# SleepingShell/verkle-kzg

Measured on AMD Instinct MI355X. Metric: width-256 commits/sec + 2^20-pt MSM ms at 1/2/4/8 GPU; achieved HBM GB/s, higher is better.
Workload: dtype u32; 1 GPU; single 2^20-point bls12_381 G1 Pippenger MSM (configs[1]); n_points=1048576, curve=bls12_381, parallelism=one GPU, exchange=none, window_bits=16, windows=7, radix=327680, radix_form=5 * 2^16, terms_per_point=2

## Files before the change

verkle-kzg_amd/csrc/ctx.hpp:

```cpp
#pragma once
#include <hip/hip_runtime.h>

#include <functional>
#include <map>
#include <memory>
#include <mutex>
#include <string>
#include <vector>

#include "../../include/vc_msm.h"

#define VK_CHECK_HIP(expr)                              \
    do {                                                \
        hipError_t e_ = (expr);                         \
        if (e_ != hipSuccess) {                         \
            vk::last_hip_error() = e_;                  \
            return e_ == hipErrorOutOfMemory ? VC_E_OOM : VC_E_HIP; \
        }                                               \
    } while (0)

#define VK_TRY(expr)            \
    do {                        \
        int s_ = (expr);        \
        if (s_ != VC_OK) return s_; \
// ... 94 lines not shown
    int win_ok = 0, win_c = 0, win_W = 0, win_ts = 0, win_m = 1;
    int win_limbs = 1;
    int win_pair = 0;
    DevBuf win;
    Table* lead = nullptr;
    int lead_k = 0, lead_c = 0;
    Table() = default;
    Table(const Table&) = delete;
    Table& operator=(const Table&) = delete;
    ~Table() { delete lead; }
};

enum WsSlot {
    WS_DIGITS = 0,
    WS_COUNTS,
    WS_OFFSETS,
    WS_CURSOR,
    WS_SORTED,
    WS_BUCKETS,
    WS_CARRY,
    WS_THROUGH,
    WS_OWNER,
    WS_OWNER_B,
    WS_SEG,
    WS_WIN,
    WS_SCAN_TMP,
    WS_SCALARS,
    WS_OUT,
    WS_MISC,
    WS_TREE,
    WS_TAIL,
    WS_PIECE,
    WS_SP_RP,
    WS_SP_COLS,
    WS_SP_SC,
    WS_SP_CNT,
    WS_SP_EOFF,
    WS_SP_OFF,
    WS_SP_ROWS,
    WS_SP_XY,
    WS_SP_INF,
    WS_SP_RC,
    WS_SP_CHUNKS,
    WS_CARRY2,
    WS_NXT,
    WS_NXT2,
    WS_CHAIN,
    WS_GLV_SC,
    WS_GLV_FLAG,
    WS_RAW_B,
    WS_SP_ITEMS,
    WS_NORM_CNT,
    WS_NORM_TOT,
    WS_COUNT_
};

struct Lane {
    hipStream_t st;
    DevBuf* ws;
    PinBuf* pin;
};

struct PendingTimer {
    hipEvent_t a, b;
    std::string name;
};

}

struct vc_ctx {
    int curve = 0;
    int device = 0;
    uint64_t uid = 0;
    hipStream_t stream = nullptr;
    hipStream_t own_stream = nullptr;
    hipStream_t side_stream = nullptr;
    std::recursive_mutex mu;
    std::vector<vk::Table*> tables;
    vk::DevBuf ws[vk::WS_COUNT_];
    vk::DevBuf ws2[vk::WS_COUNT_];
    vk::PinBuf pin[2];
    vk::PinBuf pin_io;
    vk::PinBuf pin_small;
    vk::PinBuf pin_norm;
    vk::PinBuf pin_y;
    vk::PinBuf pin_mp;
    vk::PinBuf pin_ipa;
    vk::PinBuf pin_verkle;
    vk::PinBuf pin_verkle2;
    vk::PinBuf pin_verkle_lv[2];
    vk::PinBuf pin_norm_vk;
    vk::PinBuf pin_sparse_ck;
    vk::PinBuf pin_sparse_ch;
    std::multimap<size_t, void*> pool_free;
    size_t pool_bytes = 0;
    bool timing = false;
    int opt_shared_windows = 1;
    size_t opt_msm_chunk = size_t(1) << 27;
    int opt_host_chunks = 2;
    uint32_t fb_lanes = 0;
    uint32_t small_epoch = 0;
    uint32_t tail_epoch = 0;
    uint32_t norm_vk_parity = 0;
    struct {
        int c, W, terms, m, shared;
    } plan = {0, 0, 0, 0, 0};
// ... 114 lines not shown
```

verkle-kzg_amd/csrc/msm.hip:

```cpp
#include <hip/hip_runtime.h>

#include <atomic>
#include <chrono>
#include <immintrin.h>
#include <cstdio>
#include <hipcub/hipcub.hpp>

#include <algorithm>
#include <type_traits>
#include <cstdlib>
#include <cstring>
#include <functional>
#include <mutex>
#include <set>
#include <utility>
#include <vector>

#include "ctx.hpp"
#include "host/pool.hpp"
#include "ec.hpp"
#include "msm_tail.hpp"
#include "ec29.hpp"

namespace vk {
// ... 200 lines not shown
        if (b0 + k < bins) {
            loff[b0 + k] = run;
            lcur[b0 + k] = run;
            run += counts[(size_t)(bin0 + b0 + k) * nblk + slot];
        }
    if (t == blockDim.x - 1) loff[bins] = part[t];
    __syncthreads();
    const uint32_t fmask = (1u << FB) - 1;
    const uint32_t lo = blockIdx.x * chunk, hi = min(lo + chunk, n);
    auto put = [&](uint32_t i, int w, int32_t d) {
        if (d != 0 && w >= wb) {
            const uint32_t b = (uint32_t)(d < 0 ? -d : d) - 1;
            const uint32_t p = atomicAdd(
                &lcur[(stride ? (uint32_t)w / wps : (uint32_t)(w - wb)) * NBC + (b >> FB) - bin0], 1u);
            stage[p] = sort_pack<uint32_t>(b & fmask, stride ? src.pt(i) + ((uint32_t)w % wps) * stride : i, d < 0, FB);
        }
    };
    if constexpr (std::is_same<Src, RadixDigits>::value) {
        constexpr int PRE = 4, WMAX = 8;
        if (we - src.w0 <= WMAX) {
            for (uint32_t i0 = lo + t; i0 < hi; i0 += PRE * blockDim.x) {
                int32_t dg[PRE][WMAX];
#pragma unroll
                for (int k = 0; k < PRE; k++) {
                    const uint32_t i = i0 + (uint32_t)k * blockDim.x;
#pragma unroll
                    for (int j = 0; j < WMAX; j++)
                        dg[k][j] = (i < hi && src.w0 + j < we) ? src.dig[(size_t)(src.w0 + j) * src.nv + i] : 0;
                }
#pragma unroll
                for (int k = 0; k < PRE; k++) {
                    const uint32_t i = i0 + (uint32_t)k * blockDim.x;
                    if (i >= hi) break;
#pragma unroll
                    for (int j = 0; j < WMAX; j++)
                        if (src.w0 + j < we) put(i, src.w0 + j, dg[k][j]);
                }
            }
        } else {
            for (uint32_t i = lo + t; i < hi; i += blockDim.x) src(i, c, we, [&](int w, int32_t d) { put(i, w, d); });
        }
    } else {
        for (uint32_t i = lo + t; i < hi; i += blockDim.x) src(i, c, we, [&](int w, int32_t d) { put(i, w, d); });
    }
    __syncthreads();
    const uint32_t grp = t >> 4, sub = t & 15, ngrp = blockDim.x >> 4;
    for (uint32_t g = grp; g < bins; g += ngrp) {
        const uint32_t l0 = loff[g], len = loff[g + 1] - l0;
        const uint32_t gb = base[(size_t)(bin0 + g) * nblk + slot];
        for (uint32_t j = sub; j < len; j += 16) tmp[gb + j] = stage[l0 + j];
    }
}

template <class T>
__global__ void __launch_bounds__(1024) k_sort_fine(const T* __restrict__ tmp, const uint32_t* __restrict__ base,
                                                   uint32_t nblk, uint32_t bins, uint32_t FB,
                                                   uint32_t* __restrict__ offsets, uint32_t* __restrict__ sorted,
                                                   uint32_t* __restrict__ zero_word, uint32_t cap, uint32_t regs_ok) {
    __shared__ uint32_t h[256], x[256];
    extern __shared__ uint32_t stage[];
    const uint32_t g = blockIdx.x, F = 1u << FB, t = threadIdx.x;
    const bool cnt_lane = t < 256;
    if (zero_word != nullptr && g == 0 && t == 0) *zero_word = 0;
    const uint32_t start = base[(size_t)g * nblk];
    const uint32_t end = base[(size_t)(g + 1) * nblk];
    if (cnt_lane) h[t] = 0;
    __syncthreads();
    constexpr uint32_t RMAX = 16;
    T er[RMAX];
    const bool regs = regs_ok != 0 && cap != 0 && end - start <= cap && end - start <= RMAX * blockDim.x;
    if (regs) {
#pragma unroll
        for (uint32_t k = 0; k < RMAX; k++) {
            const uint32_t p = start + t + k * blockDim.x;
            er[k] = p < end ? tmp[p] : T(0);
        }
#pragma unroll
        for (uint32_t k = 0; k < RMAX; k++)
            if (start + t + k * blockDim.x < end) atomicAdd(&h[sort_fine_of<T>(er[k], FB)], 1u);
    } else {
        constexpr uint32_t RH = 4;
        for (uint32_t p0 = start + t; p0 < end; p0 += RH * blockDim.x) {
            T e[RH];
#pragma unroll
            for (uint32_t k = 0; k < RH; k++) {
                const uint32_t p = p0 + k * blockDim.x;
                e[k] = p < end ? tmp[p] : T(0);
            }
#pragma unroll
            for (uint32_t k = 0; k < RH; k++)
                if (p0 + k * blockDim.x < end) atomicAdd(&h[sort_fine_of<T>(e[k], FB)], 1u);
        }
    }
    __syncthreads();
    const uint32_t v = cnt_lane ? h[t] : 0u;
    if (cnt_lane) x[t] = v;
    __syncthreads();
    for (uint32_t o = 1; o < 256; o <<= 1) {
        const uint32_t a = (cnt_lane && t >= o) ? x[t - o] : 0u;
        __syncthreads();
        if (cnt_lane) x[t] += a;
        __syncthreads();
    }
    const uint32_t excl = cnt_lane ? x[t] - v : 0u;
    if (t < F) offsets[(size_t)g * F + t] = start + excl;
    if (g == bins - 1 && t == 0) offsets[(size_t)bins * F] = end;
    __syncthreads();
    if (cnt_lane) h[t] = excl;
    __syncthreads();
    constexpr uint32_t RS = 4;
    if (regs) {
#pragma unroll
        for (uint32_t k = 0; k < RMAX; k++)
            if (start + t + k * blockDim.x < end) stage[atomicAdd(&h[sort_fine_of<T>(er[k], FB)], 1u)] = sort_entry_of<T>(er[k], FB);
        __syncthreads();
        for (uint32_t p = t; p < end - start; p += blockDim.x) sorted[start + p] = stage[p];
        return;
    }
    if (end - start <= cap) {
        for (uint32_t p0 = start + t; p0 < end; p0 += RS * blockDim.x) {
            T e[RS];
            uint32_t pos[RS];
#pragma unroll
            for (uint32_t k = 0; k < RS; k++) {
                const uint32_t p = p0 + k * blockDim.x;
                e[k] = p < end ? tmp[p] : T(0);
            }
#pragma unroll
            for (uint32_t k = 0; k < RS; k++)
                if (p0 + k * blockDim.x < end) pos[k] = atomicAdd(&h[sort_fine_of<T>(e[k], FB)], 1u);
#pragma unroll
            for (uint32_t k = 0; k < RS; k++)
                if (p0 + k * blockDim.x < end) stage[pos[k]] = sort_entry_of<T>(e[k], FB);
        }
        __syncthreads();
        for (uint32_t p = t; p < end - start; p += blockDim.x) sorted[start + p] = stage[p];
        return;
    }
    for (uint32_t p0 = start + t; p0 < end; p0 += RS * blockDim.x) {
        T e[RS];
        uint32_t pos[RS];
#pragma unroll
        for (uint32_t k = 0; k < RS; k++) {
            const uint32_t p = p0 + k * blockDim.x;
            e[k] = p < end ? tmp[p] : T(0);
        }
#pragma unroll
        for (uint32_t k = 0; k < RS; k++)
            if (p0 + k * blockDim.x < end) pos[k] = start + atomicAdd(&h[sort_fine_of<T>(e[k], FB)], 1u);
#pragma unroll
        for (uint32_t k = 0; k < RS; k++)
            if (p0 + k * blockDim.x < end) sorted[pos[k]] = sort_entry_of<T>(e[k], FB);
    }
}

template <class FC, class BT, class = void>
struct is_affn : std::false_type {};
template <class FC, class BT>
struct is_affn<FC, BT, std::void_t<typename FC::AffN>> : std::is_same<BT, typename FC::AffN> {};
template <class FC, class BT, class = void>
struct is_affp : std::false_type {};
template <class FC, class BT>
struct is_affp<FC, BT, std::void_t<typename FC::AffP>> : std::is_same<BT, typename FC::AffP> {};
template <class C, class BT>
struct is_fbe : std::is_same<BT, FbE<C>> {};

static uint32_t acc_merge() {
    static const uint32_t v = getenv("VKZG_ACC_MERGE") ? (uint32_t)atoi(getenv("VKZG_ACC_MERGE")) : 0u;
    return v;
}

template <class T>
__device__ __forceinline__ T shfl_down1(const T& v) {
    static_assert(sizeof(T) % 4 == 0, "");
    constexpr int NW = (int)(sizeof(T) / 4);
    uint32_t w[NW];
    __builtin_memcpy(w, &v, sizeof w);
#pragma unroll
    for (int k = 0; k < NW; k++) w[k] = (uint32_t)__shfl_down((int)w[k], 1);
    T r;
    __builtin_memcpy(&r, w, sizeof w);
    return r;
}

template <class C, class BT = typename C::Aff>
__global__ void __launch_bounds__(256) VK_ACC_OCC k_msm_accumulate(
    const BT* __restrict__ bases, const BT* __restrict__ phi, uint32_t nphi,
    const uint32_t* __restrict__ sorted, const uint32_t* __restrict__ offsets, uint32_t NBtot, uint32_t M,
    typename Fast29<C>::type::Acc* __restrict__ buckets, typename Fast29<C>::type::Acc* __restrict__ carry_in,
    uint8_t* __restrict__ through, typename Fast29<C>::type::Acc* __restrict__ owner_piece,
    uint32_t* __restrict__ owner_bucket, uint32_t* __restrict__ chain_max, uint32_t merge,
    unsigned long long* __restrict__ clk) {
    using FC = typename Fast29<C>::type;
    using Aff = BT;
    uint32_t t = blockIdx.x * blockDim.x + threadIdx.x;
    const uint32_t L = offsets[NBtot];
    uint32_t k = t * M;
    if (k >= L) return;
    const bool stamp = clk != nullptr && t == 0;
    if (stamp) {
        clk[0] = __builtin_amdgcn_s_memtime();
        clk[1] = __builtin_amdgcn_s_memrealtime();
    }
    uint32_t e = min(k + M, L);
    owner_bucket[t] = NONE;
    through[t] = 0;
    uint32_t lo = 0, hi = NBtot;
    while (hi - lo > 1) {
        uint32_t mid = (lo + hi) >> 1;
        if (offsets[mid] <= k) lo = mid;
        else hi = mid;
    }
    uint32_t b = lo;
    uint32_t bend = offsets[b + 1];
    bool left_open = offsets[b] < k;
    typename FC::Acc acc = FC::zero();
    auto base_of = [&](uint32_t j) -> const Aff* { return j < nphi ? bases + j : phi + (j - nphi); };
    constexpr bool SN = is_affn<FC, BT>::value;
    constexpr bool SP = is_affp<FC, BT>::value;
    constexpr bool FBE = is_fbe<C, BT>::value;
    using Pre = std::conditional_t<SN || SP || FBE, typename FC::Aff, Aff>;
    auto fetch = [&](uint32_t id) -> Pre {
        if constexpr (FBE) {
            return base_of(id & 0x7fffffffu)->u;
        } else if constexpr (SP) {
            const Aff* r = bases + 2 * (size_t)(id & 0x7fffffffu) + (id >> 31);
            typename FC::Aff a;
            a.x = r->x;
            a.y = r->y;
            return a;
        } else {
            const Aff* b = base_of(id & 0x7fffffffu);
            if constexpr (SN) {
                typename FC::Aff a;
                a.x = b->x;
                a.y = *reinterpret_cast<const decltype(a.y)*>(reinterpret_cast<const char*>(&b->y) +
                                                              ((id >> 31) ? sizeof(a.y) : 0u));
                return a;
            } else {
                return *b;
            }
        }
    };
    uint32_t idx = sorted[k];
    Pre P = fetch(idx);
    uint32_t my_through = 0, own_b = NONE;
    while (true) {
        uint32_t cur = idx;
        typename FC::Aff Q;
        if constexpr (SN || SP || FBE) Q = P;
        else Q = FC::load(&P);
        if (k + 1 < e) {
            idx = sorted[k + 1];
            P = fetch(idx);
        }
        acc = FC::madd(acc, Q, !SN && !SP && (cur >> 31) != 0);
        k++;
        if (k == bend || k == e) {
            bool right_open = (k == e) && (bend > e);
            if (!left_open && !right_open) {
                buckets[b] = acc;
            } else if (left_open) {
                carry_in[t] = acc;
                my_through = right_open ? 2 : 1;
                through[t] = (uint8_t)my_through;
                if (!right_open) {
                    const uint32_t L = t - offsets[b] / M;
                    if (L >= 2) atomicMax(chain_max, L);
                }
            } else {
                owner_piece[t] = acc;
                owner_bucket[t] = b;
                own_b = b;
            }
            if (k == e) break;
            left_open = false;
            acc = FC::zero();
            do {
                b++;
                bend = offsets[b + 1];
            } while (bend <= k);
        }
    }
    if (stamp) {
        clk[2] = __builtin_amdgcn_s_memtime();
        clk[3] = __builtin_amdgcn_s_memrealtime();
    }
#ifdef VKZG_ACC_MERGE_BUILD
    if (merge) {
        const typename FC::Acc mine = my_through == 1 ? carry_in[t] : FC::zero();
        const typename FC::Acc nxt = shfl_down1(mine);
        const uint32_t nth = (uint32_t)__shfl_down((int)my_through, 1);
        if (own_b != NONE && (threadIdx.x & 63u) != 63u && nth == 1) {
            buckets[own_b] = FC::add(acc, nxt);
            owner_bucket[t] = NONE;
        }
    }
#else
    (void)merge;
    (void)my_through;
    (void)own_b;
#endif
}

template <class C>
__global__ void __launch_bounds__(256) k_fast_store(const FAcc<C>* __restrict__ a, uint32_t n,
                                                   const uint32_t* __restrict__ offsets, typename C::Acc* __restrict__ o) {
    const uint32_t i = blockIdx.x * blockDim.x + threadIdx.x;
    if (i < n && offsets[i + 1] > offsets[i]) o[i] = Fast29<C>::type::store(a[i]);
}

template <class C>
__global__ void __launch_bounds__(256) k_to_fast(const typename C::Aff* __restrict__ in, size_t n,
                                                typename C::Aff* __restrict__ out) {
    const size_t i = (size_t)blockIdx.x * blockDim.x + threadIdx.x;
    if (i >= n) return;
    Fast29<C>::type::pack_aff(in[i], out + i);
}
template <class C>
__global__ void __launch_bounds__(256) k_to_limbs(const typename C::Aff* __restrict__ in, size_t n,
                                                 typename Fast29<C>::type::Aff* __restrict__ out) {
    using FC = typename Fast29<C>::type;
    const size_t i = (size_t)blockIdx.x * blockDim.x + threadIdx.x;
    if (i >= n) return;
    typename C::Aff packed;
    FC::pack_aff(in[i], &packed);
    out[i] = FC::load(&packed);
}

template <class C>
__global__ void __launch_bounds__(256) k_to_limbs_n(const typename C::Aff* __restrict__ in, size_t n,
                                                   typename Fast29<C>::type::AffN* __restrict__ out) {
    using FC = typename Fast29<C>::type;
    const size_t i = (size_t)blockIdx.x * blockDim.x + threadIdx.x;
// ... 399 lines not shown
    t->win_pair = (pair && !packed) ? 1 : 0;
    VK_TRY(t->win.ensure((size_t)W * 2 * n * (packed ? sizeof(Aff) : t->win_pair ? 2 * sizeof(FP) : sizeof(FA))));
    Table cur;
    DevBuf nxt, acc;
    VK_TRY(nxt.ensure(n * sizeof(Aff)));
    VK_TRY(acc.ensure(n * sizeof(Acc)));
    FA* win = t->win.as<FA>();
    const unsigned g = (unsigned)((n + 255) / 256);
    for (int w = 0; w < W; w++) {
        const Aff* src = t->bases.as<Aff>();
        if (w > 0) {
            VK_LAUNCH(ctx, "win_next", (k_win_next<C>), g, 256, 0, w == 1 ? t->bases.as<Aff>() : cur.bases.as<Aff>(),
                      t->inf.as<uint8_t>(), (uint32_t)n, w == W - 1 ? c - ts : c, mul, acc.as<Acc>());
            VK_TRY(table_from_acc(ctx, &cur, acc.p, n));
            src = cur.bases.as<Aff>();
        }
        VK_LAUNCH(ctx, "glv_phi", (k_glv_phi<C>), g, 256, 0, src, (uint32_t)n, bls_fq_mont(GLV_BETA), nxt.as<Aff>());
        if (packed) {
            Aff* wp = t->win.as<Aff>();
            VK_LAUNCH(ctx, "to_fast", (k_to_fast<C>), g, 256, 0, src, n, wp + (size_t)w * 2 * n);
            VK_LAUNCH(ctx, "to_fast", (k_to_fast<C>), g, 256, 0, nxt.as<Aff>(), n, wp + (size_t)w * 2 * n + n);
        } else if (t->win_pair) {
            FP* wp = t->win.as<FP>();
            VK_LAUNCH(ctx, "to_limbs", (k_to_limbs_p<C>), g, 256, 0, src, n, wp + 2 * ((size_t)w * 2 * n));
            VK_LAUNCH(ctx, "to_limbs", (k_to_limbs_p<C>), g, 256, 0, nxt.as<Aff>(), n, wp + 2 * ((size_t)w * 2 * n + n));
        } else {
            VK_LAUNCH(ctx, "to_limbs", (k_to_limbs_n<C>), g, 256, 0, src, n, win + (size_t)w * 2 * n);
            VK_LAUNCH(ctx, "to_limbs", (k_to_limbs_n<C>), g, 256, 0, nxt.as<Aff>(), n, win + (size_t)w * 2 * n + n);
        }
    }
    VK_CHECK_HIP(hipStreamSynchronize(ctx->stream));
    t->win_ok = 1;
    t->win_c = c;
    t->win_W = W;
    t->win_ts = ts;
    t->win_m = (int)mul;
    return VC_OK;
}

static int coarse_st_lds_attr(const void* fn, int device) {
    static std::mutex mu;
    static std::set<std::pair<const void*, int>> done;
    std::lock_guard<std::mutex> lk(mu);
    if (done.count({fn, device})) return VC_OK;
    VK_CHECK_HIP(hipFuncSetAttribute(fn, hipFuncAttributeMaxDynamicSharedMemorySize, 152 * 1024));
    done.insert({fn, device});
    return VC_OK;
}

template <class Src>
static int sort_entries(vc_ctx* ctx, Lane L, Src src, uint32_t nv, int c, int wb, int we, uint32_t FB,
                        uint32_t NBC, uint32_t nblk, uint32_t chunk, uint32_t stride, uint32_t wps, size_t ncnt,
                        uint32_t* counts, uint32_t* base, void* tmp, uint32_t* offsets, uint32_t* sorted,
                        uint32_t* zero_word, bool coarse_stage = false, bool counts_ready = false,
                        uint32_t sets_split = 1) {
    hipStream_t st = L.st;
    if (stride && wps == 0) return VC_E_INVALID;
    const uint32_t bins = (stride ? ((uint32_t)we + wps - 1) / wps : (uint32_t)(we - wb)) * NBC;
    const size_t lds = (size_t)bins * 4;
    if (lds > 64 * 1024) return VC_E_INVALID;
    if (ncnt != (size_t)bins * nblk + 1) return VC_E_INVALID;
    const uint64_t emax = stride ? (uint64_t)std::min<uint32_t>((uint32_t)we, wps) * stride : (uint64_t)nv;
    const bool narrow = emax <= (1ull << (31 - FB));
    const uint32_t sblk = chunk >= 4096 ? 1024 : 256;
    if (!counts_ready)
        VK_LAUNCH_ON(ctx, st, "msm_sort_hist", (k_sort_hist<Src>), nblk, sblk, lds, src, nv, c, wb, we, FB, NBC,
                     nblk, stride, wps, chunk, counts);
    size_t tmp_bytes = 0;
    VK_CHECK_HIP(hipcub::DeviceScan::ExclusiveSum(nullptr, tmp_bytes, counts, base, ncnt, st));
    VK_TRY(L.ws[WS_SCAN_TMP].ensure(tmp_bytes));
    {
        hipEvent_t ev = nullptr;
        if (ctx->timing) ctx->timer_begin("msm_scan", &ev, st);
        VK_CHECK_HIP(hipcub::DeviceScan::ExclusiveSum(L.ws[WS_SCAN_TMP].p, tmp_bytes, counts, base, ncnt, st));
        if (ctx->timing) ctx->timer_end("msm_scan", ev, st);
    }
    static const int fine_env = getenv("VKZG_SORT_FINE_BLOCK") ? atoi(getenv("VKZG_SORT_FINE_BLOCK")) : 0;
    const uint64_t total = (uint64_t)nv * (uint32_t)(we - wb);
    int fblk = fine_env == 256 || fine_env == 1024 ? fine_env : (total / bins >= (1u << 15) ? 1024 : 256);
    static const int stage_env = getenv("VKZG_SORT_STAGE") ? atoi(getenv("VKZG_SORT_STAGE")) : 1;
    static const uint32_t fine_regs = !(getenv("VKZG_SORT_FINE_REGS") && atoi(getenv("VKZG_SORT_FINE_REGS")) == 0);
    uint32_t cap = 0;
    if (stage_env && total / bins <= 12000) {
        cap = 16384;
        if (fine_env == 0) fblk = 1024;
    }
    const uint32_t nsplit = (stride && sets_split > 1 && wb == 0 && (uint32_t)we == sets_split * wps) ? sets_split : 1;
    const uint32_t bins_l = bins / nsplit;
    const uint32_t wl = (uint32_t)(we - wb) / nsplit;
    const size_t st_lds = ((size_t)2 * bins_l + 1 + (size_t)chunk * wl) * 4;
    const bool staged = coarse_stage && narrow && st_lds <= 152 * 1024;
    if (staged) {
        VK_TRY(coarse_st_lds_attr(reinterpret_cast<const void*>(&k_sort_coarse_st<Src>), ctx->device));
        for (uint32_t s = 0; s < nsplit; s++) {
            Src ss = src;
            const int wbs = nsplit > 1 ? (int)(s * wps) : wb, wes = nsplit > 1 ? (int)((s + 1) * wps) : we;
            if constexpr (std::is_same<Src, RadixDigits>::value) ss.w0 = wbs;
            VK_LAUNCH_ON(ctx, st, "msm_sort_coarse", k_sort_coarse_st<Src>, nblk, 1024, st_lds, ss, nv, c, wbs, wes, FB,
                         NBC, nblk, stride, wps, chunk, counts, base, static_cast<uint32_t*>(tmp), s * bins_l, bins_l);
        }
        VK_LAUNCH_ON(ctx, st, "msm_sort_fine", k_sort_fine<uint32_t>, bins, fblk, cap * 4,
                     static_cast<const uint32_t*>(tmp), base, nblk, bins, FB, offsets, sorted, zero_word, cap, fine_regs);
    } else if (narrow) {
        VK_LAUNCH_ON(ctx, st, "msm_sort_coarse", (k_sort_coarse<Src, uint32_t>), nblk, sblk, lds, src, nv, c, wb, we,
                     FB, NBC, nblk, stride, wps, chunk, base, static_cast<uint32_t*>(tmp));
        VK_LAUNCH_ON(ctx, st, "msm_sort_fine", k_sort_fine<uint32_t>, bins, fblk, cap * 4,
                     static_cast<const uint32_t*>(tmp), base, nblk, bins, FB, offsets, sorted, zero_word, cap, fine_regs);
    } else {
        VK_LAUNCH_ON(ctx, st, "msm_sort_coarse", (k_sort_coarse<Src, uint64_t>), nblk, sblk, lds, src, nv, c, wb, we,
                     FB, NBC, nblk, stride, wps, chunk, base, static_cast<uint64_t*>(tmp));
        VK_LAUNCH_ON(ctx, st, "msm_sort_fine", k_sort_fine<uint64_t>, bins, fblk, cap * 4,
                     static_cast<const uint64_t*>(tmp), base, nblk, bins, FB, offsets, sorted, zero_word, cap, fine_regs);
    }
    return VC_OK;
}

static bool win_pair_on() {
    static const int env = getenv("VKZG_WIN_PAIR") ? atoi(getenv("VKZG_WIN_PAIR")) : 1;
    return env != 0;
}

static int glv_window(size_t nv) {
    if (nv >= (1u << 19)) return 16;
    if (nv >= (1u << 15)) return 13;
    return 10;
}
static int glv_window_shared(size_t nv) {
    static const int env = getenv("VKZG_MSM_C") ? atoi(getenv("VKZG_MSM_C")) : 0;
    if (env >= 8 && env <= 20) return env;
    return glv_window(nv);
}
static int top_shortfall(int c, int total) {
    const int W = (total + c - 1) / c;
    return c - (total - c * (W - 1));
}
static int choose_window(size_t n, int total) {
    int c0 = 5;
    if (n >= (1u << 19)) c0 = 16;
    else if (n >= (1u << 17)) c0 = 15;
    else if (n >= (1u << 15)) c0 = 13;
    else if (n >= (1u << 12)) c0 = 11;
    else if (n >= (1u << 9)) c0 = 9;
    else if (n >= 64) c0 = 7;
    static const int env = getenv("VKZG_MSM_TOPFIT") ? atoi(getenv("VKZG_MSM_TOPFIT")) : 1;
    if (!env || top_shortfall(c0, total) <= 2) return c0;
    int best = c0;
    double best_cost = 0.0;
    for (int c = std::max(4, c0 - 5); c <= std::min(16, c0 + 2); c++) {
        if (top_shortfall(c, total) > 2) continue;
        const double W = (total + c - 1) / c;
        const double cost = W * (double)n + 2.0 * W * (double)(1u << (c - 1));
        if (best == c0 || cost < best_cost) best = c, best_cost = cost;
    }
    return best;
}

template <class C>
struct MsmSlice {
    using Acc = typename C::Acc;
    Lane L{};
    int c = 0, wb = 0, we = 0, W = 0;
    bool shared = false;
    int top_f = 0;
    uint32_t m = 1;
    int sets = 1;
// ... 60 lines not shown
    const bool resid_sets = sl.shared || Wr <= 8;
    const uint32_t nU = (Lseg > 1 && resid_sets && (resid_env == 1 || (resid_env == 2 && sl.shared))) ? Lseg : 1;
    const uint32_t Tmax = (uint32_t)((maxL + M - 1) / M);
    hipStream_t st = L.st;

    const uint32_t lgNB = (uint32_t)c - 1;
    uint32_t FB = lgNB < 8 ? lgNB : 8;
    uint32_t chunk = SORT_CHUNK;
    if (sl.m > 1) {
        FB = lgNB < 7 ? lgNB : 7;
        chunk = 8192;
    }
    static const int chunk_env = getenv("VKZG_SORT_CHUNK") ? atoi(getenv("VKZG_SORT_CHUNK")) : 0;
    static const int fb_env = getenv("VKZG_SORT_FB") ? atoi(getenv("VKZG_SORT_FB")) : 0;
    static const int cstage_env = getenv("VKZG_SORT_CSTAGE") ? atoi(getenv("VKZG_SORT_CSTAGE")) : 1;
    bool cstage = false;
    if (sl.m > 1 && sl.shared && cstage_env) {
        const uint64_t bins_l = (uint64_t)(NB >> FB);
        const uint32_t Wl = (uint32_t)W / (uint32_t)Wr;
        const uint64_t room = (152u * 1024 / 4 > 2 * bins_l + 1) ? 152u * 1024 / 4 - 2 * bins_l - 1 : 0;
        uint32_t ch = 1u << 12;
        while (ch > 1024 && (uint64_t)ch * Wl > room) ch >>= 1;
        if ((uint64_t)ch * Wl <= room) {
            chunk = ch;
            cstage = true;
        }
    }
    if (sl.m == 1 && !sl.shared && cstage_env && FB > 1 && load / (NB >> FB) > 12000) FB--;
    if (chunk_env >= 256) chunk = (uint32_t)chunk_env;
    static const int bin_lg = getenv("VKZG_SORT_BIN_LG") ? atoi(getenv("VKZG_SORT_BIN_LG")) : 16;
    while (sl.shared && sl.m == 1 && FB > 1 && (load >> bin_lg) > (size_t)(NB >> FB)) FB--;
    while (sl.shared && sl.m == 1 && FB > 1 && (NB >> FB) < 256) FB--;
    if (fb_env >= 1 && fb_env <= (int)std::min<uint32_t>(lgNB, 8)) FB = (uint32_t)fb_env;
    const uint32_t NBC = NB >> FB;
    const uint32_t nblk = (uint32_t)((nv + chunk - 1) / chunk);
    if (sl.m == 1 && cstage_env) {
        const uint64_t per_blk = (uint64_t)chunk * (uint32_t)(sl.we - sl.wb), bins_all = (uint64_t)Wr * NBC;
        const uint64_t lds_b = (2 * bins_all + 1 + per_blk) * 4;
        cstage = per_blk >= 4096 && (per_blk >= 10 * bins_all || lds_b <= 64 * 1024);
    }
    const size_t ncnt = (size_t)Wr * NBC * nblk + 1;

    DevBuf* ws = L.ws;
    VK_TRY(ws[WS_DIGITS].ensure(maxL * 8));
    VK_TRY(ws[WS_COUNTS].ensure(ncnt * 4));
    VK_TRY(ws[WS_CURSOR].ensure(ncnt * 4));
    VK_TRY(ws[WS_OFFSETS].ensure((size_t)(NBtot + 1) * 4));
    VK_TRY(ws[WS_SORTED].ensure(maxL * 4));
    VK_TRY(ws[WS_BUCKETS].ensure((size_t)NBtot * sizeof(RAcc)));
    VK_TRY(ws[WS_CARRY].ensure((size_t)(Tmax + 8) * sizeof(RAcc)));
    VK_TRY(ws[WS_THROUGH].ensure((size_t)(Tmax + 8)));
    VK_TRY(ws[WS_OWNER].ensure((size_t)(Tmax + 8) * sizeof(RAcc)));
    VK_TRY(ws[WS_OWNER_B].ensure((size_t)(Tmax + 8) * 4));
    VK_TRY(ws[WS_SEG].ensure((size_t)S * Wr * sizeof(RAcc)));
    VK_TRY(ws[WS_TREE].ensure((size_t)S * Wr * sizeof(RAcc)));
    VK_TRY(ws[WS_WIN].ensure((size_t)Wr * msm_tail_plan(S, (uint32_t)Wr, J, nU, Fast29<C>::type::quad, Lseg == 1).slots *
                             sizeof(RAcc)));
    const size_t tail_bytes = ((size_t)Wr * (J + nU) * sizeof(Acc) + 15) & ~(size_t)15;
    VK_TRY(ws[WS_TAIL].ensure(tail_bytes + 16));

    sl.NB = NB;
    sl.NBtot = NBtot;
    sl.Tmax = Tmax;
    sl.M = M;
    sl.Lseg = Lseg;
    sl.S = S;
    sl.J = J;
    sl.nU = nU;
    sl.offsets = ws[WS_OFFSETS].as<uint32_t>();
    sl.tail_bytes = tail_bytes;
    sl.chain_max = sl.chain_dst ? sl.chain_dst : reinterpret_cast<uint32_t*>(ws[WS_TAIL].as<uint8_t>() + tail_bytes);
    sl.through = ws[WS_THROUGH].as<uint8_t>();
    sl.owner_b = ws[WS_OWNER_B].as<uint32_t>();
    sl.buckets = sl.bucket_dst ? sl.bucket_dst : ws[WS_BUCKETS].as<RAcc>();
    sl.carry = ws[WS_CARRY].as<RAcc>();
    sl.owner = ws[WS_OWNER].as<RAcc>();
    sl.seg = ws[WS_SEG].as<RAcc>();
    sl.rs = ws[WS_TREE].as<RAcc>();
    sl.bsum_part = ws[WS_WIN].as<RAcc>();
    sl.tail = ws[WS_TAIL].as<Acc>();

    bool counts_ready = false;
    static const bool timing = getenv("VKZG_HOST_TIMING") && atoi(getenv("VKZG_HOST_TIMING")) != 0;
    if (timing)
        sl.t_launch0 =
            std::chrono::duration<double, std::micro>(std::chrono::steady_clock::now().time_since_epoch()).count();
    if constexpr (std::is_same<C, BLS381G1>::value) {
        if (!sl.radix.sc.empty()) {
            static const int fuse_env = getenv("VKZG_RADIX_HIST") ? atoi(getenv("VKZG_RADIX_HIST")) : 1;
            const uint32_t rn = sl.radix.n;
            const int ns = (int)sl.radix.sc.size();
            counts_ready = fuse_env && sl.shared && Wr == ns && sl.wb == 0 && (uint32_t)sl.we == sl.wps * (uint32_t)ns &&
                           nv == 2 * (size_t)rn && rn % chunk == 0 && (size_t)2 * NBC * 4 <= 64 * 1024;
            for (int s2 = 0; s2 < ns; s2++) {
                int32_t* dig = sl.radix.dig + (size_t)s2 * sl.wps * nv;
                if (counts_ready)
                    VK_LAUNCH_ON(ctx, st, "glv_split", (k_glv_radix_hist<BLS381Fr, 5, 16>), rn / chunk, 1024,
                                 (size_t)2 * NBC * 4, sl.radix.sc[s2], sl.radix.inf, rn, sl.radix.mont[s2], glv_consts(),
                                 (int)sl.wps, dig, FB, NBC, nblk, chunk, ws[WS_COUNTS].as<uint32_t>(),
                                 (uint32_t)s2 * NBC, (uint32_t)Wr * NBC);
                else
                    VK_LAUNCH_ON(ctx, st, "glv_split", (k_glv_radix<BLS381Fr, 5, 16>), (rn + 255) / 256, 256, 0,
                                 sl.radix.sc[s2], sl.radix.inf, rn, sl.radix.mont[s2], glv_consts(), (int)sl.wps, dig);
            }
        }
    }
    VK_TRY(sort_entries(ctx, L, src, (uint32_t)nv, c, sl.wb, sl.we, FB, NBC, nblk, chunk, sl.shared ? (sl.stride ? sl.stride : (uint32_t)nv) : 0u,
                        sl.wps, ncnt,
                        ws[WS_COUNTS].as<uint32_t>(),
                        ws[WS_CURSOR].as<uint32_t>(), ws[WS_DIGITS].p, sl.offsets,
                        ws[WS_SORTED].as<uint32_t>(), sl.chain_max, cstage, counts_ready,
                        sl.shared ? (uint32_t)Wr : 1u));
    if (acc_wait) VK_CHECK_HIP(hipStreamWaitEvent(st, acc_wait, 0));
    VK_LAUNCH_ON(ctx, st, "msm_accumulate", (k_msm_accumulate<C, BT>), (Tmax + 255) / 256, 256, 0, bases, phi, nphi,
                 ws[WS_SORTED].as<uint32_t>(), sl.offsets, NBtot, M, sl.buckets, sl.carry, sl.through, sl.owner,
                 sl.owner_b, sl.chain_max, acc_merge(), (unsigned long long*)ctx->clk_slot());
    if (acc_done) VK_CHECK_HIP(hipEventRecord(acc_done, st));
    sl.guard = msm_fixup_guard_rounds(sl.shared ? load : load << sl.top_f, NB, M);
    if (sl.shared) sl.guard = std::max<uint32_t>(sl.guard, 4);
    static const int fix_env = getenv("VKZG_MSM_FIXUP") ? atoi(getenv("VKZG_MSM_FIXUP")) : 0;
    if (fix_env == 1)
        VK_TRY(msm_tail_fixup<C>(ctx, L, Tmax, sl.offsets + NBtot, M, sl.buckets, sl.carry, sl.through, sl.owner,
                                 sl.owner_b, sl.chain_max, sl.guard));
    else
        VK_TRY(msm_tail_fixup_walk<C>(ctx, L, sl.offsets, NBtot, M, sl.buckets, sl.carry, sl.owner, 1u << sl.guard,
                                      sl.owner_b, sl.through, Tmax));
    if (sl.skip_reduce) return VC_OK;
    static const bool poll_env = !(getenv("VKZG_TAIL_POLL") && atoi(getenv("VKZG_TAIL_POLL")) == 0);
    TailDirect td;
    Acc* out = sl.tail;
    sl.direct = false;
    if (poll_env && L.pin->flags == hipHostMallocCoherent) {
        sl.nflags = (uint32_t)Wr * (J + nU);
        sl.flag_off = tail_bytes + 16;
        VK_TRY(L.pin->ensure(sl.flag_off + (size_t)sl.nflags * 4));
        volatile uint32_t* hf = reinterpret_cast<volatile uint32_t*>(static_cast<uint8_t*>(L.pin->p) + sl.flag_off);
        for (uint32_t k = 0; k < sl.nflags; k++) hf[k] = 0;
        sl.epoch = ++ctx->tail_epoch == 0 ? ++ctx->tail_epoch : ctx->tail_epoch;
        uint8_t* dbase = static_cast<uint8_t*>(L.pin->dp);
        td.flags = reinterpret_cast<uint32_t*>(dbase + sl.flag_off);
        td.epoch = sl.epoch;
        td.chain_src = sl.chain_max;
        td.chain_dst = reinterpret_cast<uint32_t*>(dbase + tail_bytes);
        out = reinterpret_cast<Acc*>(dbase);
        sl.direct = true;
    }
    VK_TRY(msm_tail_reduce<C>(ctx, L, sl.buckets, sl.offsets, NB, Wr, Lseg, S, J, sl.seg, sl.rs, sl.bsum_part, out,
                              nU > 1, sl.direct ? &td : nullptr));
    return VC_OK;
}

template <class C>
static int slice_fetch(MsmSlice<C>& sl) {
    sl.ht.resize((size_t)sl.Wr * (sl.J + sl.nU));
    if (sl.direct) return VC_OK;
    VK_TRY(sl.L.pin->ensure(sl.tail_bytes + 16));
    VK_CHECK_HIP(hipMemcpyAsync(sl.L.pin->p, sl.tail, sl.tail_bytes + 4, hipMemcpyDeviceToHost, sl.L.st));
    return VC_OK;
}

template <class C>
static int slice_wait(const MsmSlice<C>& sl) {
    if (sl.direct) {
        const volatile uint32_t* hf =
            reinterpret_cast<const volatile uint32_t*>(static_cast<const uint8_t*>(sl.L.pin->p) + sl.flag_off);
        const auto w0 = std::chrono::steady_clock::now();
        for (uint32_t spins = 0;; spins++) {
            uint32_t k = 0;
            while (k < sl.nflags && hf[k] == sl.epoch) k++;
// ... 682 lines not shown
        VK_CHECK_HIP(hipMemcpyAsync(d_rp.p, ch.cptr, rc_off + (batch + 1) * 4, hipMemcpyHostToDevice, st));
        rc_dev = reinterpret_cast<const uint32_t*>(d_rp.as<uint8_t>() + rc_off);
    }
    const uint32_t* d_cols = d_cols_in;
    const uint32_t* d_sc = static_cast<const uint32_t*>(d_sc_in);
    VK_TRY(ctx->ws[WS_CHAIN].ensure(4));
    uint32_t* chain_max = ctx->ws[WS_CHAIN].as<uint32_t>();
    const char* fe_env = getenv("VKZG_SPARSE_FUSED");
    const bool fused = !(fe_env && atoi(fe_env) == 0);
    if (fused) {
        DevBuf& cntb = ctx->ws[WS_NORM_CNT];
        if (cntb.p == nullptr) {
            VK_TRY(cntb.ensure(256));
            VK_CHECK_HIP(hipMemsetAsync(cntb.p, 0, 256, st));
        }
        const size_t nb = nnz / 256 + 1;
        VK_TRY(d_eoff.ensure(nb * 8 + (nb + 1) * 4));
        uint64_t* bsum = d_eoff.as<uint64_t>();
        uint32_t* boff = reinterpret_cast<uint32_t*>(bsum + nb);
        const uint32_t epoch = ++ctx->small_epoch == 0 ? ++ctx->small_epoch : ctx->small_epoch;
        VK_LAUNCH(ctx, "sparse_count_scan", (k_sparse_count_scan<Fr>), (unsigned)nb, 256, 0, d_sc, nnz, mont, fg,
                  d_cnt.as<uint32_t>(), bsum, boff, cntb.as<uint32_t>() + 16, Tmax > 0 ? chain_max : (uint32_t*)nullptr,
                  epoch);
        VK_LAUNCH(ctx, "sparse_expand_rows", (k_sparse_expand_rows<Fr, C>), (unsigned)((std::max(nnz, nch + 1) + 255) / 256),
                  256, 0, d_sc, d_cols, nnz, mont, fg, d_cnt.as<uint32_t>(), boff, d_ent.as<uint32_t>(), rp_dev, nch,
                  d_off.as<uint32_t>(), d_chunks.as<Acc>());
    } else {
        VK_CHECK_HIP(hipMemsetAsync(d_cnt.as<uint32_t>() + nnz, 0, 4, st));
        if (nnz)
            VK_LAUNCH(ctx, "sparse_count", (k_sparse_count<Fr>), (nnz + 255) / 256, 256, 0, d_sc, nnz, mont, fg,
                      d_cnt.as<uint32_t>());
        size_t tmp_bytes = 0;
        VK_CHECK_HIP(hipcub::DeviceScan::ExclusiveSum(nullptr, tmp_bytes, d_cnt.as<uint32_t>(), d_eoff.as<uint32_t>(),
                                                      nnz + 1, st));
        VK_TRY(d_tmp.ensure(std::max<size_t>(tmp_bytes, 1)));
        VK_CHECK_HIP(hipcub::DeviceScan::ExclusiveSum(d_tmp.p, tmp_bytes, d_cnt.as<uint32_t>(), d_eoff.as<uint32_t>(),
                                                      nnz + 1, st));
        if (nnz)
            VK_LAUNCH(ctx, "sparse_expand", (k_sparse_expand<Fr>), (nnz + 255) / 256, 256, 0, d_sc, d_cols, nnz, mont, fg,
                      d_eoff.as<uint32_t>(), d_ent.as<uint32_t>());
        VK_LAUNCH(ctx, "sparse_rows", (k_sparse_rows<C>), (nch + 1 + 255) / 256, 256, 0, rp_dev,
                  d_eoff.as<uint32_t>(), nch, d_off.as<uint32_t>(), d_chunks.as<Acc>());
        if (Tmax > 0) VK_CHECK_HIP(hipMemsetAsync(chain_max, 0, 4, st));
    }
    using FA = FbE<C>;
    const FA* tab = t->fb.as<FA>();
    if (Tmax > 0) {
        using RAcc = FAcc<C>;
        DevBuf& d_raw = ctx->ws[WS_RAW_B];
        VK_TRY(d_raw.ensure(nch * sizeof(RAcc)));
        VK_LAUNCH(ctx, "sparse_accumulate", (k_msm_accumulate<C, FA>), (Tmax + 255) / 256, 256, 0, tab, tab, 0xffffffffu,
                  d_ent.as<uint32_t>(), d_off.as<uint32_t>(), (uint32_t)nch, M, d_raw.as<RAcc>(), d_carry.as<RAcc>(),
                  d_thr.as<uint8_t>(), d_own.as<RAcc>(), d_ownb.as<uint32_t>(), chain_max, acc_merge(),
                  (unsigned long long*)nullptr);
        VK_TRY(msm_tail_fixup_walk<C>(ctx, ctx->lane(0), d_off.as<uint32_t>(), (uint32_t)nch, M, d_raw.as<RAcc>(),
                                      d_carry.as<RAcc>(), d_own.as<RAcc>(), 0xffffffffu, d_ownb.as<uint32_t>(),
                                      d_thr.as<uint8_t>(), Tmax));
        VK_LAUNCH(ctx, "sparse_store", (k_fast_store<C>), (nch + 255) / 256, 256, 0, d_raw.as<RAcc>(), (uint32_t)nch,
                  d_off.as<uint32_t>(), d_chunks.as<Acc>());
    }
    Acc* rows_p = d_rows.as<Acc>();
    if (ch.identity)
        rows_p = d_chunks.as<Acc>();
    else
        VK_LAUNCH(ctx, "sparse_combine", (k_sparse_combine<typename C::Inl>), batch, 64, 0, d_chunks.as<Acc>(),
                  rc_dev, rows_p);
    if constexpr (std::is_same<C, BN254G1>::value) {
        if (d_items) {
            lap("kernels");
            return normalize_rows_items(ctx, rows_p, batch, d_add_ids, d_add_xy, d_add_inf, d_dst,
                                        static_cast<uint64_t*>(d_xy), d_inf, static_cast<uint64_t*>(d_items), overlap);
        }
    }
    if (d_dst || overlap) return VC_E_INVALID;
    if (d_add_ids)
        VK_LAUNCH(ctx, "sparse_add_base", (k_rows_add_base<C>), (unsigned)((batch + 255) / 256), 256, 0,
                  rows_p, batch, d_add_ids, d_add_xy, d_add_inf);
    lap("kernels");
    VK_TRY(normalize_to_canon(ctx, ctx->curve, rows_p, batch, d_xy, d_inf));
    lap("normalise");
    if (d_items) VK_TRY(to_data_item_device(ctx, d_xy, d_inf, batch, d_items));
    return VC_OK;
}

template <class C, class Fr>
static int msm_batch_sparse_t(vc_ctx* ctx, Table* t, size_t batch, const uint64_t* row_ptr, const uint32_t* cols,
                              const uint64_t* scalars, int mont, uint64_t* out_xy, uint8_t* out_inf,
                              uint64_t* out_items = nullptr) {
    if (batch == 0) return VC_OK;
    const size_t nnz = row_ptr[batch];
    std::vector<uint8_t> bad_part(host_pool().size(), 0);
    host_pool().run([&](unsigned k) {
        const unsigned T = host_pool().size();
        uint8_t b = 0;
        for (size_t g = batch * k / T; g < batch * (k + 1) / T; g++) b |= row_ptr[g + 1] < row_ptr[g] ? 1 : 0;
        for (size_t j = nnz * k / T; j < nnz * (k + 1) / T; j++) b |= cols[j] >= t->n ? 2 : 0;
        bad_part[k] = b;
    });
    uint8_t bad = 0;
    for (uint8_t b : bad_part) bad |= b;
    if (bad & 1) return VC_E_INVALID;
    if (bad & 2) return VC_E_RANGE;
    hipStream_t st = ctx->stream;
    DevBuf& d_cols = ctx->ws[WS_SP_COLS];
    DevBuf& d_sc = ctx->ws[WS_SP_SC];
    DevBuf& d_xy = ctx->ws[WS_SP_XY];
    DevBuf& d_inf = ctx->ws[WS_SP_INF];
// ... 367 lines not shown
```

Before: 398.5 2^20-pt MSM/s.

## Precompute accumulate thread start buckets in fine sort and prefetch next indices

The fine-sort kernel now writes a per-accumulate-thread descriptor (starting bucket, its begin and end, and the next bucket's end), found by a binary search over the block's shared-memory prefix. The accumulate kernel reads this instead of doing its own binary search over the global offsets array, which removes a chain of dependent global loads at thread start. The accumulate loop also loads the sorted index two steps ahead and prefetches the next bucket boundary so bucket transitions avoid a serial offsets walk. This costs an extra workspace buffer and extra writes in the sort kernel. It also adds a few out-of-range-guarded loads per iteration.

```diff
diff --git a/verkle-kzg_amd/csrc/ctx.hpp b/verkle-kzg_amd/csrc/ctx.hpp
--- a/verkle-kzg_amd/csrc/ctx.hpp
+++ b/verkle-kzg_amd/csrc/ctx.hpp
@@ -170,6 +170,7 @@
     WS_SP_ITEMS,
     WS_NORM_CNT,
     WS_NORM_TOT,
+    WS_STARTS,
     WS_COUNT_
 };
 
diff --git a/verkle-kzg_amd/csrc/msm.hip b/verkle-kzg_amd/csrc/msm.hip
--- a/verkle-kzg_amd/csrc/msm.hip
+++ b/verkle-kzg_amd/csrc/msm.hip
@@ -276,11 +276,16 @@
     }
 }
 
+struct alignas(16) AccStart {
+    uint32_t b, begin, end, next_end;
+};
+
 template <class T>
 __global__ void __launch_bounds__(1024) k_sort_fine(const T* __restrict__ tmp, const uint32_t* __restrict__ base,
                                                    uint32_t nblk, uint32_t bins, uint32_t FB,
                                                    uint32_t* __restrict__ offsets, uint32_t* __restrict__ sorted,
-                                                   uint32_t* __restrict__ zero_word, uint32_t cap, uint32_t regs_ok) {
+                                                   uint32_t* __restrict__ zero_word, uint32_t cap, uint32_t regs_ok,
+                                                   AccStart* __restrict__ starts, uint32_t M) {
     __shared__ uint32_t h[256], x[256];
     extern __shared__ uint32_t stage[];
     const uint32_t g = blockIdx.x, F = 1u << FB, t = threadIdx.x;
@@ -329,6 +334,24 @@
     const uint32_t excl = cnt_lane ? x[t] - v : 0u;
     if (t < F) offsets[(size_t)g * F + t] = start + excl;
     if (g == bins - 1 && t == 0) offsets[(size_t)bins * F] = end;
+    if (starts != nullptr) {
+        for (uint64_t u = ((uint64_t)start + M - 1) / M + t; u * M < end; u += blockDim.x) {
+            const uint32_t rel = (uint32_t)(u * M) - start;
+            uint32_t lo = 0, hi = F - 1;
+            while (lo < hi) {
+                const uint32_t mid = (lo + hi) >> 1;
+                if (x[mid] > rel) hi = mid;
+                else lo = mid + 1;
+            }
+            AccStart r;
+            r.b = g * F + lo;
+            r.begin = start + (lo ? x[lo - 1] : 0u);
+            r.end = start + x[lo];
+            r.next_end = lo + 1 < F ? start + x[lo + 1] : 0u;
+            starts[u] = r;
+        }
+        if (g == bins - 1 && t == 0) starts[((uint64_t)end + M - 1) / M] = AccStart{bins * F, end, end, 0u};
+    }
     __syncthreads();
     if (cnt_lane) h[t] = excl;
     __syncthreads();
@@ -414,7 +437,7 @@
     typename Fast29<C>::type::Acc* __restrict__ buckets, typename Fast29<C>::type::Acc* __restrict__ carry_in,
     uint8_t* __restrict__ through, typename Fast29<C>::type::Acc* __restrict__ owner_piece,
     uint32_t* __restrict__ owner_bucket, uint32_t* __restrict__ chain_max, uint32_t merge,
-    unsigned long long* __restrict__ clk) {
+    unsigned long long* __restrict__ clk, const AccStart* __restrict__ starts) {
     using FC = typename Fast29<C>::type;
     using Aff = BT;
     uint32_t t = blockIdx.x * blockDim.x + threadIdx.x;
@@ -429,15 +452,26 @@
     uint32_t e = min(k + M, L);
     owner_bucket[t] = NONE;
     through[t] = 0;
-    uint32_t lo = 0, hi = NBtot;
-    while (hi - lo > 1) {
-        uint32_t mid = (lo + hi) >> 1;
-        if (offsets[mid] <= k) lo = mid;
-        else hi = mid;
-    }
-    uint32_t b = lo;
-    uint32_t bend = offsets[b + 1];
-    bool left_open = offsets[b] < k;
+    uint32_t b, bbeg, bend, nxt;
+    if (starts != nullptr) {
+        const AccStart s = starts[t];
+        b = s.b;
+        bbeg = s.begin;
+        bend = s.end;
+        nxt = s.next_end;
+    } else {
+        uint32_t lo = 0, hi = NBtot;
+        while (hi - lo > 1) {
+            uint32_t mid = (lo + hi) >> 1;
+            if (offsets[mid] <= k) lo = mid;
+            else hi = mid;
+        }
+        b = lo;
+        bbeg = offsets[b];
+        bend = offsets[b + 1];
+        nxt = 0;
+    }
+    uint32_t left_open = t - bbeg / M;
     typename FC::Acc acc = FC::zero();
     auto base_of = [&](uint32_t j) -> const Aff* { return j < nphi ? bases + j : phi + (j - nphi); };
     constexpr bool SN = is_affn<FC, BT>::value;
@@ -467,6 +501,7 @@
         }
     };
     uint32_t idx = sorted[k];
+    uint32_t idx2 = sorted[min(k + 1, e - 1)];
     Pre P = fetch(idx);
     uint32_t my_through = 0, own_b = NONE;
     while (true) {
@@ -474,10 +509,9 @@
         typename FC::Aff Q;
         if constexpr (SN || SP || FBE) Q = P;
         else Q = FC::load(&P);
-        if (k + 1 < e) {
-            idx = sorted[k + 1];
-            P = fetch(idx);
-        }
+        idx = idx2;
+        idx2 = sorted[min(k + 2, e - 1)];
+        P = fetch(idx);
         acc = FC::madd(acc, Q, !SN && !SP && (cur >> 31) != 0);
         k++;
         if (k == bend || k == e) {
@@ -488,22 +522,25 @@
                 carry_in[t] = acc;
                 my_through = right_open ? 2 : 1;
                 through[t] = (uint8_t)my_through;
-                if (!right_open) {
-                    const uint32_t L = t - offsets[b] / M;
-                    if (L >= 2) atomicMax(chain_max, L);
-                }
+                if (!right_open && left_open >= 2) atomicMax(chain_max, left_open);
             } else {
                 owner_piece[t] = acc;
                 owner_bucket[t] = b;
                 own_b = b;
             }
             if (k == e) break;
-            left_open = false;
+            left_open = 0;
             acc = FC::zero();
-            do {
+            if (nxt > k) {
                 b++;
-                bend = offsets[b + 1];
-            } while (bend <= k);
+                bend = nxt;
+            } else {
+                do {
+                    b++;
+                    bend = offsets[b + 1];
+                } while (bend <= k);
+            }
+            nxt = offsets[min(b + 2, NBtot)];
         }
     }
     if (stamp) {
@@ -1009,8 +1046,8 @@
 static int sort_entries(vc_ctx* ctx, Lane L, Src src, uint32_t nv, int c, int wb, int we, uint32_t FB,
                         uint32_t NBC, uint32_t nblk, uint32_t chunk, uint32_t stride, uint32_t wps, size_t ncnt,
                         uint32_t* counts, uint32_t* base, void* tmp, uint32_t* offsets, uint32_t* sorted,
-                        uint32_t* zero_word, bool coarse_stage = false, bool counts_ready = false,
-                        uint32_t sets_split = 1) {
+                        uint32_t* zero_word, AccStart* starts, uint32_t M, bool coarse_stage = false,
+                        bool counts_ready = false, uint32_t sets_split = 1) {
     hipStream_t st = L.st;
     if (stride && wps == 0) return VC_E_INVALID;
     const uint32_t bins = (stride ? ((uint32_t)we + wps - 1) / wps : (uint32_t)(we - wb)) * NBC;
@@ -1057,17 +1094,20 @@
                          NBC, nblk, stride, wps, chunk, counts, base, static_cast<uint32_t*>(tmp), s * bins_l, bins_l);
         }
         VK_LAUNCH_ON(ctx, st, "msm_sort_fine", k_sort_fine<uint32_t>, bins, fblk, cap * 4,
-                     static_cast<const uint32_t*>(tmp), base, nblk, bins, FB, offsets, sorted, zero_word, cap, fine_regs);
+                     static_cast<const uint32_t*>(tmp), base, nblk, bins, FB, offsets, sorted, zero_word, cap, fine_regs,
+                     starts, M);
     } else if (narrow) {
         VK_LAUNCH_ON(ctx, st, "msm_sort_coarse", (k_sort_coarse<Src, uint32_t>), nblk, sblk, lds, src, nv, c, wb, we,
                      FB, NBC, nblk, stride, wps, chunk, base, static_cast<uint32_t*>(tmp));
         VK_LAUNCH_ON(ctx, st, "msm_sort_fine", k_sort_fine<uint32_t>, bins, fblk, cap * 4,
-                     static_cast<const uint32_t*>(tmp), base, nblk, bins, FB, offsets, sorted, zero_word, cap, fine_regs);
+                     static_cast<const uint32_t*>(tmp), base, nblk, bins, FB, offsets, sorted, zero_word, cap, fine_regs,
+                     starts, M);
     } else {
         VK_LAUNCH_ON(ctx, st, "msm_sort_coarse", (k_sort_coarse<Src, uint64_t>), nblk, sblk, lds, src, nv, c, wb, we,
                      FB, NBC, nblk, stride, wps, chunk, base, static_cast<uint64_t*>(tmp));
         VK_LAUNCH_ON(ctx, st, "msm_sort_fine", k_sort_fine<uint64_t>, bins, fblk, cap * 4,
-                     static_cast<const uint64_t*>(tmp), base, nblk, bins, FB, offsets, sorted, zero_word, cap, fine_regs);
+                     static_cast<const uint64_t*>(tmp), base, nblk, bins, FB, offsets, sorted, zero_word, cap, fine_regs,
+                     starts, M);
     }
     return VC_OK;
 }
@@ -1234,6 +1274,8 @@
     VK_TRY(ws[WS_THROUGH].ensure((size_t)(Tmax + 8)));
     VK_TRY(ws[WS_OWNER].ensure((size_t)(Tmax + 8) * sizeof(RAcc)));
     VK_TRY(ws[WS_OWNER_B].ensure((size_t)(Tmax + 8) * 4));
+    VK_TRY(ws[WS_STARTS].ensure((size_t)(Tmax + 8) * sizeof(AccStart)));
+    AccStart* const starts = ws[WS_STARTS].as<AccStart>();
     VK_TRY(ws[WS_SEG].ensure((size_t)S * Wr * sizeof(RAcc)));
     VK_TRY(ws[WS_TREE].ensure((size_t)S * Wr * sizeof(RAcc)));
     VK_TRY(ws[WS_WIN].ensure((size_t)Wr * msm_tail_plan(S, (uint32_t)Wr, J, nU, Fast29<C>::type::quad, Lseg == 1).slots *
@@ -1291,12 +1333,12 @@
                         sl.wps, ncnt,
                         ws[WS_COUNTS].as<uint32_t>(),
                         ws[WS_CURSOR].as<uint32_t>(), ws[WS_DIGITS].p, sl.offsets,
-                        ws[WS_SORTED].as<uint32_t>(), sl.chain_max, cstage, counts_ready,
+                        ws[WS_SORTED].as<uint32_t>(), sl.chain_max, starts, M, cstage, counts_ready,
                         sl.shared ? (uint32_t)Wr : 1u));
     if (acc_wait) VK_CHECK_HIP(hipStreamWaitEvent(st, acc_wait, 0));
     VK_LAUNCH_ON(ctx, st, "msm_accumulate", (k_msm_accumulate<C, BT>), (Tmax + 255) / 256, 256, 0, bases, phi, nphi,
                  ws[WS_SORTED].as<uint32_t>(), sl.offsets, NBtot, M, sl.buckets, sl.carry, sl.through, sl.owner,
-                 sl.owner_b, sl.chain_max, acc_merge(), (unsigned long long*)ctx->clk_slot());
+                 sl.owner_b, sl.chain_max, acc_merge(), (unsigned long long*)ctx->clk_slot(), starts);
     if (acc_done) VK_CHECK_HIP(hipEventRecord(acc_done, st));
     sl.guard = msm_fixup_guard_rounds(sl.shared ? load : load << sl.top_f, NB, M);
     if (sl.shared) sl.guard = std::max<uint32_t>(sl.guard, 4);
@@ -2085,7 +2127,7 @@
         VK_LAUNCH(ctx, "sparse_accumulate", (k_msm_accumulate<C, FA>), (Tmax + 255) / 256, 256, 0, tab, tab, 0xffffffffu,
                   d_ent.as<uint32_t>(), d_off.as<uint32_t>(), (uint32_t)nch, M, d_raw.as<RAcc>(), d_carry.as<RAcc>(),
                   d_thr.as<uint8_t>(), d_own.as<RAcc>(), d_ownb.as<uint32_t>(), chain_max, acc_merge(),
-                  (unsigned long long*)nullptr);
+                  (unsigned long long*)nullptr, (const AccStart*)nullptr);
         VK_TRY(msm_tail_fixup_walk<C>(ctx, ctx->lane(0), d_off.as<uint32_t>(), (uint32_t)nch, M, d_raw.as<RAcc>(),
                                       d_carry.as<RAcc>(), d_own.as<RAcc>(), 0xffffffffu, d_ownb.as<uint32_t>(),
                                       d_thr.as<uint8_t>(), Tmax));
```

New measurement: 411.4 2^20-pt MSM/s, median of 6. 1.03x the previous value.
